# AdvancedPhotonSource/tike

Hardware: AMD Instinct MI355X
Metric: diffraction patterns/sec/GPU (256x256, 8-mode probe) (higher is better)
Workload: dtype c64; 1 GPU; c3; positions_per_gpu=10000, modes=8, detector=256, eigen_probes=1, solver=lstsq_grad, num_batch=10, chunk_positions=1000, position_correction=False, object_update=after every minibatch (batch_method wobbly_center), route=no_farplane

## Files before the change

include/tike_amd.h:

```cpp
#ifndef TIKE_AMD_H
#define TIKE_AMD_H

#ifdef __cplusplus
extern "C" {
#endif

#define TIKE_ERR_ARG 1000001
#define TIKE_ERR_UNSUPPORTED 1000002
#define TIKE_ERR_COMM 2000000
#define TIKE_COMM_ID_BYTES 128

#define TIKE_ABI_VERSION 14

const char* tike_build_id(void);

int tike_abi_version(void);

int tike_set_deterministic(int on, void* scratch, long bytes);

int tike_init(void);

int tike_patch_fwd(const void* images, void* patches, const float* positions, int nimage, int H,
                   int W, int nscan, int nrepeat, int patch_width, int padded_width,
                   void* stream);
int tike_patch_adj(void* images, const void* patches, const float* positions, int nimage, int H,
                   int W, int nscan, int nrepeat, int patch_width, int padded_width, int npatch,
                   void* stream);

int tike_conv_fwd(const void* psi, const float* scan, const void* probe, int probe_per_scan,
                  void* nearplane, int nscan, int S, int pw, int det, int H, int W, void* stream);
int tike_conv_adj(const void* nearplane, const float* scan, const void* probe,
                  int probe_per_scan, void* psi, int nscan, int S, int pw, int det, int H, int W,
                  void* stream);
int tike_conv_adj_probe(const void* nearplane, const float* scan, const void* psi,
                        void* probe_adj, int nscan, int S, int pw, int det, int H, int W,
                        void* stream);

int tike_fft2(const void* in, void* out, long ntile, int n, int inverse, float scale,
              void* stream);

int tike_fft2_supported(int n);

int tike_fft2_general(const void* in, void* out, long ntile, int n, int inverse, float scale,
                      int lines_per_group_rows, int lines_per_group_cols, void* stream);

int tike_ptycho_fwd(const void* psi, const float* scan, const void* probe, int probe_per_scan,
                    const void* eigen_probe, const float* eigen_weights, int num_eigen,
                    int eigen_modes, void* farplane, int nscan, int S, int pw, int det, int H,
                    int W, float scale, int sub_batch, void* stream);

int tike_ptycho_adj(const void* farplane, const void* probe, int probe_per_scan,
                    const float* scan, const void* psi, void* psi_adj, void* probe_adj,
                    void* objproj_work, float* acc_work, int nscan, int S, int pw, int det,
                    int H, int W, float scale, int sub_batch, void* stream);

int tike_ptycho_fwd_intensity(const void* psi, const float* scan, const void* probe,
                              int probe_per_scan, const void* unique_probe,
                              const float* eigen_weights, int num_eigen, int eigen_modes,
                              void* farplane, float* intensity, void* patches, int nscan, int S,
                              int pw, int det, int H, int W, float scale, void* stream);

int tike_ptycho_fwd_intensity_only(const void* psi, const float* scan, const void* probe,
                                   int probe_per_scan, const void* unique_probe,
                                   const float* eigen_weights, int num_eigen, int eigen_modes,
                                   void* scratch, float* intensity, int nscan, int S, int pw,
// ... 279 lines not shown
                                  const void* other, const float* scan, const void* data,
                                  int data_u16, void* far_a, int a_valid, void* far_b,
                                  float* costs_k, int nscan, int chunk, int S, int det, int H,
                                  int W, float fwd_scale, double count, double* state,
                                  int stage, double* sums, void* stream);

int tike_cgrad_line_search_linear_masked(int variable, const void* x, const void* d, void* xs,
                                         const void* other, const float* scan, const void* data,
                                         int data_u16, void* far_a, int a_valid, void* far_b,
                                         float* costs_k, int nscan, int chunk, int S, int det,
                                         int H, int W, float fwd_scale, double count,
                                         double* state, int stage, double* sums,
                                         const unsigned char* measured, int model,
                                         long num_measured, void* stream);

int tike_eigen_pixel_update1(const void* patches, const void* chi0, const void* mpu0,
                             const void* eigen0, const float* eigen_proj,
                             const float* weights_c, long weights_row, const float* norm,
                             void* update, int nscan, int pw, int chi_modes, const float* stats,
                             const float* costs, float eps, float* sums3, const void* psi,
                             const float* scan, int H, int W, void* stream);
int tike_lstsq_tail_mid(void* eigen0, const void* update, int npix, float* nacc,
                        float beta_eigen, const float* stats, int B, float eps,
                        const float* sums3, double count, int recover_psi, int recover_probe,
                        float* tail3, void* stream);
int tike_eigen_position_sums1(const void* patches, const void* chi0, const void* mpu0,
                              const void* eigen0, float* sums5, float* dsum, int nscan, int pw,
                              int chi_modes, const void* psi, const float* scan, int H, int W,
                              void* stream);
int tike_lstsq_tail_finish(const float* tail3, const float* sums3, double count, float* steps,
                           void* probe, void* combined, const void* mpu, float inv_num_batch,
                           long nprobe, float* weights, long weights_row, int S, int m,
                           const float* stats, const float* sums5, int B, int npix,
                           void* stream);

int tike_ifft2_pass2_gradients_eproj(const void* work, const void* patches, const void* probe,
                                     const void* eigen_probe, const float* eigen_weights,
                                     int num_eigen, int eigen_modes, void* objproj, void* chi0,
                                     void* m_probe_update, float mpu_scale, int nscan, int S,
                                     int det, float inv_scale, float* qtab, float* q,
                                     void* stream);
int tike_eigen_pixel_update1q(const void* patches, const void* chi0, const void* mpu0,
                              const void* eigen0, const float* q, const float* weights_c,
                              long weights_row, const float* norm, void* update, int nscan,
                              int pw, int chi_modes, const void* psi, const float* scan, int H,
                              int W, float* c0part, float* eproj_out, void* stream);
int tike_lstsq_step_stats_eigen1(const void* chi, const float* scan,
                                 const void* object_update_precond, const void* probe,
                                 const void* eigen_probe, const float* eigen_weights,
                                 int eigen_modes, const void* m_probe_update, const void* patches,
                                 const void* update, float* nacc, double count, float beta_eigen,
                                 float* stats, float* sums5, int nscan, int S, int chi_modes,
                                 int pw, int H, int W, void* stream);
int tike_lstsq_tail_solve1(void* eigen0, const void* update, int npix, const float* nacc,
                           float beta_eigen, const float* stats, const float* costs,
                           const float* sums5, int B, float eps, double count, int recover_psi,
                           int recover_probe, float* sums3, float* tail3, void* stream);

int tike_lstsq_chunk_gradients(const void* psi, const float* scan, const void* probe,
                               const void* eigen_probe, const float* eigen_weights,
                               int num_eigen, int eigen_modes, const void* data, int data_u16,
                               const unsigned char* measured, int model,
                               float unmeasured_scaling, long num_measured, void* scratch,
                               void* work, float* gscale, void* patches, float* costs,
                               void* objproj, void* chi0, void* m_probe_update,
                               float mpu_scale, float* object_acc, int nscan, int S, int det,
                               int H, int W, float fwd_scale, float inv_scale, void* stream);

int tike_comm_unique_id(void* id);
int tike_comm_create(const void* id, int nranks, int rank, void** comm);
int tike_comm_destroy(void* comm);
int tike_comm_allreduce_sum(void* comm, void* buf, long count, int f64, void* stream);
int tike_comm_broadcast(void* comm, void* buf, long nbytes, int root, void* stream);

int tike_cluster_farthest_fill(const float* points, long n, long* owner, int num_cluster,
                               long turns);
int tike_cluster_swap_sweep(const double* dist, long n, int k, long* label, const long* best,
                            const long* order, double* regret, int* moved);

#ifdef __cplusplus
}
#endif
#endif
```

tike_amd/_lib.py:

```python
import ctypes
import os
import re

import torch

_HERE = os.path.dirname(os.path.abspath(__file__))
LIB_PATH = os.environ.get("TIKE_AMD_LIB") or os.path.join(
    _HERE, "csrc", "libtike_amd.so")
HEADER_PATH = os.path.join(os.path.dirname(_HERE), "include", "tike_amd.h")

ABI_VERSION = 14
ERR_ARG = 1000001
ERR_UNSUPPORTED = 1000002
ERR_COMM = 2000000
COMM_ID_BYTES = 128

if not os.path.isfile(LIB_PATH):
    raise ImportError(
        f"{LIB_PATH} not found: build the HIP library first "
        "(`make -C tike_amd/csrc` or `python -c 'import __graft_entry__ as g; "
        "g.build()'`). tike_amd has no CPU fallback.")

lib = ctypes.CDLL(LIB_PATH)

_p = ctypes.c_void_p
_i = ctypes.c_int
_l = ctypes.c_long
_f = ctypes.c_float
_d = ctypes.c_double

_PROTOTYPES = {
    "tike_abi_version": [],
    "tike_init": [],
    "tike_set_deterministic": [_i, _p, _l],
    "tike_patch_fwd": [_p, _p, _p, _i, _i, _i, _i, _i, _i, _i, _p],
    "tike_patch_adj": [_p, _p, _p, _i, _i, _i, _i, _i, _i, _i, _i, _p],
    "tike_conv_fwd": [_p, _p, _p, _i, _p, _i, _i, _i, _i, _i, _i, _p],
    "tike_conv_adj": [_p, _p, _p, _i, _p, _i, _i, _i, _i, _i, _i, _p],
    "tike_conv_adj_probe": [_p, _p, _p, _p, _i, _i, _i, _i, _i, _i, _p],
    "tike_fft2": [_p, _p, _l, _i, _i, _f, _p],
    "tike_fft2_supported": [_i],
    "tike_fft2_general": [_p, _p, _l, _i, _i, _f, _i, _i, _p],
    "tike_pfa_supported": [_i, _i, _i],
    "tike_pfa_fwd_gather": [_p, _p, _p, _i, _p, _p, _p, _i, _i, _p, _p, _i, _i, _i,
                            _i, _i, _i, _p],
    "tike_pfa_fwd_subtiles_supported": [_i, _i, _i],
    "tike_pfa_fwd_subtiles": [_p, _p, _p, _p, _p, _i, _i, _p, _p, _p, _i, _i,
                              _i, _i, _i, _i, _p],
    "tike_pfa_fft2": [_p, _p, _l, _i, _i, _p],
    "tike_pfa_combine_gradient": [_p, _p, _p, _p, _i, _i, _i, _f, _i, _f, _l, _i,
                                  _p],
    "tike_pfa_inv_products": [_p, _p, _p, _i, _p, _p, _p, _i, _i, _p, _p, _p, _f,
                              _i, _i, _i, _i, _f, _p],
    "tike_gen_supported": [_i, _i, _i],
    "tike_gen_fwd_rows": [_p, _p, _p, _i, _p, _p, _p, _i, _i, _p, _p, _i, _i, _i,
                          _i, _i, _i, _p],
    "tike_gen_cols_gradient": [_p, _p, _p, _p, _p, _i, _i, _i, _i, _f, _i, _f,
                               _l, _p],
    "tike_gen_inv_rows_gradients": [_p, _p, _p, _i, _p, _p, _p, _i, _i, _p, _p,
                                    _p, _f, _i, _i, _i, _i, _f, _p],
    "tike_fresnel_spect_prop": [_p, _p, _p, _l, _i, _i, _f, _f, _p],
    "tike_fft2_pass1": [_p, _p, _l, _i, _i, _p],
    "tike_fft2_pass2_inplace": [_p, _l, _i, _i, _f, _p],
    "tike_slice_step": [_p, _p, _p, _p, _i, _i, _i, _i, _i, _f, _p],
# ... 39 lines not shown
    "tike_ifft2_pass2_gradients_modes": [_p, _p, _p, _p, _p, _i, _i, _p, _p,
                                         _p, _f, _i, _i, _i, _f, _i, _i, _i, _p],
    "tike_poisson_steps_grad_ifft2_pass1": [_p, _p, _i, _p, _p, _p, _p, _p, _i,
                                            _i, _i, _f, _f, _l, _f, _f, _p],
    "tike_object_update_precond": [_p, _p, _p, _f, _p, _p, _p, _l, _p],
    "tike_lstsq_step_sums": [_p, _p, _i, _f, _p, _p],
    "tike_lstsq_step_solve": [_p, _i, _f, _p, _d, _i, _i, _p, _p],
    "tike_probe_update": [_p, _p, _p, _p, _f, _l, _p],
    "tike_eigen_weights0": [_p, _p, _i, _i, _i, _i, _p, _p],
    "tike_eigen_proj_mean": [_p, _i, _p, _l, _p, _l, _i, _p, _p],
    "tike_eigen_normalise": [_p, _p, _d, _f, _i, _p, _p, _p],
    "tike_eigen_dsum": [_p, _i, _l, _p, _p],
    "tike_eigen_weights": [_p, _i, _l, _p, _d, _p, _l, _p, _i, _p, _p],
    "tike_grad_ifft2_crop": [_p, _p, _p, _p, _i, _p, _p, _l, _i, _i, _f, _f,
                             _p],
    "tike_position_sums": [_p, _p, _i, _p, _p, _p, _i, _i, _p, _i, _p, _p, _i,
                           _i, _i, _p],
    "tike_rpie_position_sums": [_p, _p, _p, _p, _i, _p, _p, _i, _i, _p, _i, _p,
                                _p, _p, _i, _i, _i, _i, _i, _p],
    "tike_farplane_gradient": [_p, _p, _p, _p, _p, _i, _i, _i, _i, _i, _f, _l,
                               _p],
    "tike_intensity": [_p, _p, _l, _i, _l, _p],
    "tike_cost_each_pattern": [_p, _p, _p, _l, _l, _i, _p],
    "tike_objective_grad": [_p, _p, _p, _p, _l, _i, _l, _i, _p],
    "tike_lstsq_gradients": [_p, _p, _p, _p, _p, _p, _i, _i, _p, _p, _p, _p, _i,
                             _i, _i, _i, _i, _p],
    "tike_varying_probe": [_p, _p, _p, _i, _i, _p, _i, _i, _i, _p],
    "tike_scatter_patches": [_p, _p, _p, _i, _i, _i, _i, _p],
    "tike_eigen_position_sums": [_p, _p, _p, _p, _p, _i, _i, _i, _p, _i, _i,
                                 _i, _p],
    "tike_eigen_pixel_update": [_p, _p, _p, _p, _p, _i, _i, _i, _p, _p, _i, _i,
                                _i, _p],
    "tike_probe_grad": [_p, _p, _p, _p, _p, _i, _i, _i, _i, _i, _p],
    "tike_probe_preconditioner": [_p, _p, _p, _i, _i, _i, _i, _p],
    "tike_psi_preconditioner": [_p, _p, _p, _i, _i, _i, _i, _p],
    "tike_scatter_amplitudes": [_p, _p, _p, _i, _i, _i, _i, _p],
    "tike_lstsq_step_stats": [_p, _p, _p, _p, _p, _p, _p, _i, _i, _p, _p, _p,
                              _p, _i, _i, _i, _i, _i, _i, _p, _p, _p],
    "tike_eigen_pixel_update1": [_p, _p, _p, _p, _p, _p, _l, _p, _p, _i, _i, _i,
                                 _p, _p, _f, _p, _p, _p, _i, _i, _p],
    "tike_lstsq_tail_mid": [_p, _p, _i, _p, _f, _p, _i, _f, _p, _d, _i, _i, _p,
                            _p],
    "tike_eigen_position_sums1": [_p, _p, _p, _p, _p, _p, _i, _i, _i, _p, _p,
                                  _i, _i, _p],
    "tike_lstsq_tail_finish": [_p, _p, _d, _p, _p, _p, _p, _f, _l, _p, _l, _i,
                               _i, _p, _p, _i, _i, _p],
    "tike_ifft2_pass2_gradients_eproj": [_p, _p, _p, _p, _p, _i, _i, _p, _p,
                                         _p, _f, _i, _i, _i, _f, _p, _p, _p],
    "tike_eigen_pixel_update1q": [_p, _p, _p, _p, _p, _p, _l, _p, _p, _i, _i,
                                  _i, _p, _p, _i, _i, _p, _p, _p],
    "tike_lstsq_step_stats_eigen1": [_p, _p, _p, _p, _p, _p, _i, _p, _p, _p,
                                     _p, _d, _f, _p, _p, _i, _i, _i, _i, _i,
                                     _i, _p],
    "tike_lstsq_tail_solve1": [_p, _p, _i, _p, _f, _p, _p, _p, _i, _f, _d, _i,
                               _i, _p, _p, _p],
    "tike_lstsq_chunk_gradients": [_p, _p, _p, _p, _p, _i, _i, _p, _i, _p, _i,
                                   _f, _l, _p, _p, _p, _p, _p, _p, _p, _p, _f,
                                   _p, _i, _i, _i, _i, _i, _f, _f, _p],
    "tike_cgrad_direction": [_p, _p, _p, _p, _l, _i, _p, _i, _d, _p, _p, _p],
    "tike_cgrad_line_search": [_i, _p, _p, _p, _p, _p, _p, _i, _p, _p, _i, _i,
                               _i, _i, _i, _i, _f, _d, _p, _p, _i, _p],
    "tike_cgrad_line_search_linear": [_i, _p, _p, _p, _p, _p, _p, _i, _p, _i, _p,
                                      _p, _i, _i, _i, _i, _i, _i, _f, _d, _p, _i,
                                      _p, _p],
    "tike_cgrad_line_search_masked": [_i, _p, _p, _p, _p, _p, _p, _i, _p, _p,
                                      _i, _i, _i, _i, _i, _i, _f, _d, _p, _p,
                                      _i, _p, _i, _l, _p],
    "tike_cgrad_line_search_linear_masked": [_i, _p, _p, _p, _p, _p, _p, _i, _p,
                                             _i, _p, _p, _i, _i, _i, _i, _i, _i,
                                             _f, _d, _p, _i, _p, _p, _i, _l, _p],
    "tike_comm_unique_id": [_p],
    "tike_comm_create": [_p, _i, _i, ctypes.POINTER(_p)],
    "tike_comm_destroy": [_p],
    "tike_comm_allreduce_sum": [_p, _p, _l, _i, _p],
    "tike_comm_broadcast": [_p, _p, _l, _i, _p],
    "tike_cluster_farthest_fill": [_p, _l, _p, _i, _l],
    "tike_cluster_swap_sweep": [_p, _l, _i, _p, _p, _p, _p, _p],
}


def build_id():
    try:
        fn = lib.tike_build_id
    except AttributeError:
        return ""
    fn.restype = ctypes.c_char_p
    fn.argtypes = []
    return fn().decode()


def declared_symbols():
    with open(HEADER_PATH) as f:
        text = f.read()
    return sorted(set(re.findall(r"^int\s+(tike_\w+)\s*\(", text, flags=re.M)))


for _name, _args in _PROTOTYPES.items():
    try:
        _fn = getattr(lib, _name)
    except AttributeError as e:
        raise ImportError(
            f"{LIB_PATH} does not export {_name}: it was built from another "
            "include/tike_amd.h; rebuild it (`make -C tike_amd/csrc`).") from e
    _fn.argtypes = _args
    _fn.restype = ctypes.c_int

# ... 48 lines not shown
```

tike_amd/csrc/lstsq.hip:

```cpp
#include "fft_engine2.h"
#include <type_traits>

#include "internal.h"
#include "tike_amd.h"

#ifndef TK_STATS_PAIRS
#define TK_STATS_PAIRS 1
#endif
static const bool g_stats_pairs = TK_STATS_PAIRS != 0;

constexpr int TK_STRIP = 32;
#define TK_ATOMIC_ADD(p, v) unsafeAtomicAdd(p, v)

template <bool REAL_ONLY, class ValueFn, class Sink>
__device__ __forceinline__ void scatter_footprint_rows(ValueFn&& value, float fx, float fy,
                                                       int pw, int r0, int r1, Sink&& sink) {
  for (int x0 = 0; x0 < pw; x0 += blockDim.x) {
    const int xp = x0 + threadIdx.x;
    const bool active = xp < pw;
    cf uprev = mk(0.f, 0.f), uprev_last = mk(0.f, 0.f);
    constexpr int RG = 4;
    cf vv[RG], ll[RG], nv[RG], nl[RG];
    auto load_group = [&](int yb, cf (&a)[RG], cf (&b)[RG]) {
      const int xpc = active ? xp : pw - 1;
// ... 1812 lines not shown
  auto taps16 = [&](const unsigned off) {
    tk_v4f t;
    __builtin_memcpy(&t, reinterpret_cast<const char*>(psi) + off, sizeof(t));
    return t;
  };
  auto tap = [](const tk_v4f u, const tk_v4f l, const TkCorner& c) {
    cf o = mk(u.x * c.w00, u.y * c.w00);
    o.x += u.z * c.w01;
    o.y += u.w * c.w01;
    o.x += l.x * c.w10;
    o.y += l.y * c.w10;
    o.x += l.z * c.w11;
    o.y += l.w * c.w11;
    return o;
  };
  for (int pair = blockIdx.x; pair < npair; pair += gridDim.x) {
    const int n0 = 2 * pair;
    const bool two = n0 + 1 < nscan;
    const TkCorner c0 = tk_corner(scan, n0);
    const TkCorner c1 = tk_corner(scan, two ? n0 + 1 : n0);
    const bool in0 = tk_interior(c0, pw, H, W), in1 = tk_interior(c1, pw, H, W);
    if (!(two && in0 && in1)) {
      one(n0, c0, in0);
      if (two) one(n0 + 1, c1, in1);
      continue;
    }
    float a[5] = {0.f, 0.f, 0.f, 0.f, 0.f}, b[5] = {0.f, 0.f, 0.f, 0.f, 0.f};
    const unsigned base0 = (unsigned)(c0.sy * W + c0.sx), base1 = (unsigned)(c1.sy * W + c1.sx);
    const cf* __restrict__ chi_a = R.chi0 + (long)n0 * R.XS;
    const cf* __restrict__ chi_b = chi_a + R.XS;
    const int ybeg = ((int)threadIdx.x / cols) * rows;
    for (int x = (int)threadIdx.x % cols; x < pw; x += 256) {
      unsigned rel = (unsigned)(ybeg * W + x);
      tk_v4f u0 = taps16((base0 + rel) * 8u), u1 = taps16((base1 + rel) * 8u);
      int p = ybeg * pw + x;
#pragma unroll 2
      for (int y = 0; y < rows; ++y) {
        rel += (unsigned)W;
        const tk_v4f l0 = taps16((base0 + rel) * 8u), l1 = taps16((base1 + rel) * 8u);
        const cf e = E[p], m0 = R.mpu0[p];
        const cf xa = chi_a[p], xb = chi_b[p];
        add(a, tap(u0, l0, c0), xa, e, m0);
        add(b, tap(u1, l1, c1), xb, e, m0);
        u0 = l0;
        u1 = l1;
        p += pw;
      }
    }
    finish(a, n0);
    finish(b, n0 + 1);
  }
}

__global__ __launch_bounds__(256) __attribute__((amdgpu_waves_per_eu(4)))
void step_stats_eigen_pair_kernel(
    const cf* __restrict__ chi, const float* __restrict__ scan, const cf* __restrict__ gobj,
    const TkProbe probe, const cf* __restrict__ mpu, const cf* __restrict__ patches,
    const cf* __restrict__ update, const float* __restrict__ nacc, float inv_count, float beta,
    float* __restrict__ stats, float* __restrict__ sums5, int nscan, int chi_modes, int pw,
    int H, int W, int nsplit) {
  __shared__ float red[4];
  typedef float tk_v4f __attribute__((ext_vector_type(4)));
  const long P = (long)pw * pw;
  const int plen = (int)(P / nsplit);
  const int npair = (nscan + 1) / 2;
  const float uu = nacc[0], ee = nacc[1], eu = nacc[2];
  const float mu = sqrtf(uu * inv_count * inv_count / (float)P);
  const float kk = beta / mu * inv_count;
  const float inv = 1.0f / sqrtf((ee + 2.0f * kk * eu + kk * kk * uu) / (float)P);
  auto enew = [&](const cf e, const long p) { return (e + update[p] * kk) * inv; };
  auto esum = [](float* a, const cf o, const cf x, const cf e, const cf m0) {
    const cf r = conjf(o) * x - m0;
    const cf phi = o * e;
    a[0] += r.x * e.x + r.y * e.y;
    a[1] += x.x * phi.x + x.y * phi.y;
    a[2] += norm2(phi);
    a[3] += r.y * e.x - r.x * e.y;
  };
  auto put = [&](float* dst, const float v) {
    if (nsplit > 1)
      unsafeAtomicAdd(dst, v);
    else
      *dst = v;
  };
  auto finish5 = [&](const float* a, const int n) {
    float t[4];
#pragma unroll
    for (int k = 0; k < 4; ++k) t[k] = tk_block_sum256(a[k], red);
    if (threadIdx.x == 0) {
      float* o = sums5 + (long)n * 5;
      put(o, t[0]);
      put(o + 1, t[1]);
      put(o + 2, t[2]);
      put(o + 3, t[0]);
      put(o + 4, t[3]);
    }
  };
  for (int v = blockIdx.x; v < npair * nsplit; v += gridDim.x) {
    const int n0 = 2 * (v / nsplit), part = v % nsplit;
    const TkCorner c0 = tk_corner(scan, n0);
    const bool two = n0 + 1 < nscan;
    const TkCorner c1 = tk_corner(scan, two ? n0 + 1 : n0);
    const bool in0 = c0.sy >= 0 && c0.sx >= 0 && c0.sy + pw < H && c0.sx + pw < W;
    const bool in1 = c1.sy >= 0 && c1.sx >= 0 && c1.sy + pw < H && c1.sx + pw < W;
    const int pbeg = part * plen + (int)threadIdx.x;
    const int pend = part + 1 == nsplit ? (int)P : (part + 1) * plen;
    if (!(two && in0 && in1)) {
      for (int i = 0; i < (two ? 2 : 1); ++i) {
        const int n = n0 + i;
        step_stats_item<true, true>(chi, scan, nullptr, gobj, probe, mpu, patches, stats,
                                    chi_modes, pw, H, W, nullptr, nullptr, nsplit, n, part, red);
        float a[4] = {0.f, 0.f, 0.f, 0.f};
        for (int p = pbeg; p < pend; p += blockDim.x)
          esum(a, patches[(long)n * P + p], chi[(long)n * chi_modes * P + p],
               enew(probe.eigen[p], p), mpu[p]);
        finish5(a, n);
      }
      continue;
    }
    float s0 = 1.0f, s1 = 1.0f, t0 = 0.f, t1 = 0.f;
    if (probe.weights != nullptr) {
      const float* w = probe.weights + n0 * (long)(probe.C + 1) * probe.S;
      s0 = w[0];
      s1 = w[(long)(probe.C + 1) * probe.S];
      t0 = w[probe.S];
      t1 = w[(long)(probe.C + 1) * probe.S + probe.S];
    }
    float a[8] = {0.f, 0.f, 0.f, 0.f, 0.f, 0.f, 0.f, 0.f};
    float b[8] = {0.f, 0.f, 0.f, 0.f, 0.f, 0.f, 0.f, 0.f};
    float ea[4] = {0.f, 0.f, 0.f, 0.f}, eb[4] = {0.f, 0.f, 0.f, 0.f};
    const unsigned base0 = (unsigned)(c0.sy * W + c0.sx), base1 = (unsigned)(c1.sy * W + c1.sx);
    const cf* __restrict__ chi_a = chi + ((long)n0 * chi_modes) * P;
    const cf* __restrict__ chi_b = chi + ((long)(n0 + 1) * chi_modes) * P;
    const cf* __restrict__ pat_a = patches + (long)n0 * P;
    const cf* __restrict__ pat_b = pat_a + P;
    auto tap = [](const tk_v4f u, const tk_v4f l, const TkCorner& c) {
      cf g = mk(u.x * c.w00, u.y * c.w00);
      g.x += u.z * c.w01;
      g.y += u.w * c.w01;
      g.x += l.x * c.w10;
      g.y += l.y * c.w10;
      g.x += l.z * c.w11;
      g.y += l.w * c.w11;
      return g;
    };
    auto sums = [](float* acc, const cf g, const cf o, const cf x0, const cf p0, const cf pn,
                   const cf m0) {
      const cf dOP = g * pn;
      const cf dPO = m0 * o;
      const cf OP = o * p0;
      acc[0] += norm2(dOP);
      acc[1] += norm2(dPO);
      const cf a2 = dOP * conjf(dPO);
      acc[2] += a2.x;
      acc[3] += a2.y;
      acc[4] += dOP.x * x0.x + dOP.y * x0.y;
      acc[5] += dPO.x * x0.x + dPO.y * x0.y;
      acc[6] += OP.x * x0.x + OP.y * x0.y;
      acc[7] += norm2(OP);
    };
    auto pixel = [&](const int p, const tk_v4f u0, const tk_v4f l0, const tk_v4f u1,
                     const tk_v4f l1) {
      const cf oa = pat_a[p], ob = pat_b[p];
      const cf xa = chi_a[p], xb = chi_b[p];
      const cf p0 = probe.probe[p];
      const cf m0 = mpu[p];
      const cf e1 = probe.eigen[p];
      const cf en = enew(e1, p);
      cf pa = p0 * s0, pb = p0 * s1;
      pa.x += t0 * e1.x;
      pa.y += t0 * e1.y;
      pb.x += t1 * e1.x;
      pb.y += t1 * e1.y;
      sums(a, tap(u0, l0, c0), oa, xa, p0, pa, m0);
      sums(b, tap(u1, l1, c1), ob, xb, p0, pb, m0);
      esum(ea, oa, xa, en, m0);
      esum(eb, ob, xb, en, m0);
    };
    auto taps16 = [&](const unsigned off) {
      tk_v4f t;
      __builtin_memcpy(&t, reinterpret_cast<const char*>(gobj) + off, sizeof(t));
      return t;
    };
    const int cols = pw < 256 ? pw : 256, groups = 256 / cols;
    const int rows = pw / (nsplit * groups);
    const int ybeg = (part * groups + (int)threadIdx.x / cols) * rows;
    for (int x = (int)threadIdx.x % cols; x < pw; x += 256) {
      unsigned rel = (unsigned)(ybeg * W + x);
      tk_v4f u0 = taps16((base0 + rel) * 8u), u1 = taps16((base1 + rel) * 8u);
      int p = ybeg * pw + x;
#pragma unroll 2
      for (int y = 0; y < rows; ++y) {
        rel += (unsigned)W;
        const tk_v4f l0 = taps16((base0 + rel) * 8u), l1 = taps16((base1 + rel) * 8u);
        pixel(p, u0, l0, u1, l1);
        u0 = l0;
        u1 = l1;
        p += pw;
      }
    }
#pragma unroll
    for (int k = 0; k < 8; ++k) {
      const float ta = tk_block_sum256(a[k], red);
      const float tb = tk_block_sum256(b[k], red);
      if (threadIdx.x == 0) {
        put(&stats[(long)n0 * 8 + k], ta);
        put(&stats[(long)n0 * 8 + 8 + k], tb);
      }
    }
    finish5(ea, n0);
    finish5(eb, n0 + 1);
  }
}

__global__ __launch_bounds__(256) void eigen_norm_sums1_kernel(const cf* __restrict__ E,
                                                               const cf* __restrict__ update,
                                                               int npix, float* __restrict__ nacc,
                                                               float* __restrict__ part) {
  __shared__ float red[4];
  float uu = 0.f, ee = 0.f, eu = 0.f;
  for (int i = blockIdx.x * 256 + threadIdx.x; i < npix; i += gridDim.x * 256) {
    const cf e = E[i], u = update[i];
    uu += norm2(u);
    ee += norm2(e);
    eu += e.x * u.x + e.y * u.y;
  }
  uu = tk_block_sum256(uu, red);
  ee = tk_block_sum256(ee, red);
  eu = tk_block_sum256(eu, red);
  if (threadIdx.x == 0) {
    if (part != nullptr) {
      part[3 * blockIdx.x] = uu;
      part[3 * blockIdx.x + 1] = ee;
      part[3 * blockIdx.x + 2] = eu;
    } else {
      unsafeAtomicAdd(&nacc[0], uu);
      unsafeAtomicAdd(&nacc[1], ee);
      unsafeAtomicAdd(&nacc[2], eu);
    }
  }
}

extern "C" int tike_lstsq_step_stats_eigen1(const void* chi, const float* scan,
                                            const void* object_update_precond, const void* probe,
                                            const void* eigen_probe, const float* eigen_weights,
                                            int eigen_modes, const void* m_probe_update,
                                            const void* patches, const void* update, float* nacc,
                                            double count, float beta_eigen, float* stats,
                                            float* sums5, int nscan, int S, int chi_modes,
                                            int pw, int H, int W, void* stream) {
  TK_ENTER();
  TK_CHECK_ARG(nscan >= 0 && S >= 1 && chi_modes >= 1 && pw >= 1 && H >= 1 && W >= 1 &&
               eigen_modes >= 1 && count > 0);
  TK_CHECK_ARG(probe && eigen_probe && eigen_weights && m_probe_update && update && nacc);
  const long P = (long)pw * pw;
  const long nitem = (nscan + 1) / 2;
  int nsplit = 1;
  while (nsplit < 16 && nitem * nsplit * 2 <= 8192 && P % (2048L * nsplit) == 0) nsplit *= 2;
  if (tk_deterministic()) nsplit = 1;
  const int groups = 256 / (pw < 256 ? pw : 256);
  if (!((pw % 256 == 0 || 256 % pw == 0) && pw % (nsplit * groups) == 0 &&
        (long)H * W < (1L << 28)))
    return TK_ERR_UNSUPPORTED;
  int grid = P >= 256 * 64 ? 64 : (int)((P + 255) / 256);
  float* part = nullptr;
  if (tk_deterministic()) {
    part = tk_det_scratch(sizeof(float) * 3 * (size_t)grid);
    if (part == nullptr) grid = 1;
  }
  hipLaunchKernelGGL(eigen_norm_sums1_kernel, dim3(grid), dim3(256), 0, (hipStream_t)stream,
                     (const cf*)eigen_probe, (const cf*)update, (int)P, nacc, part);
  TK_LAUNCH_CHECK();
  if (part != nullptr) {
    int rc = tk_ordered_sum(nacc, part, 3, grid, true, (hipStream_t)stream);
    if (rc) return rc;
  }
  if (nscan == 0) return TK_OK;
  TK_CHECK_ARG(chi && scan && object_update_precond && patches && stats && sums5);
  const TkProbe pr = tk_make_probe(probe, 0, eigen_probe, eigen_weights, 1, eigen_modes, S, pw,
                                   nullptr);
  if (nsplit > 1) {
    hipError_t e = hipMemsetAsync(stats, 0, sizeof(float) * 8 * (size_t)nscan, (hipStream_t)stream);
    if (e == hipSuccess)
      e = hipMemsetAsync(sums5, 0, sizeof(float) * 5 * (size_t)nscan, (hipStream_t)stream);
    if (e != hipSuccess) return (int)e;
  }
  hipLaunchKernelGGL(step_stats_eigen_pair_kernel, dim3(tk_grid(nitem * nsplit, 16)), dim3(256),
                     0, (hipStream_t)stream, (const cf*)chi, scan,
                     (const cf*)object_update_precond, pr, (const cf*)m_probe_update,
                     (const cf*)patches, (const cf*)update, (const float*)nacc,
                     (float)(1.0 / count), beta_eigen, stats, sums5, nscan, chi_modes, pw, H, W,
                     nsplit);
  TK_LAUNCH_CHECK();
  return TK_OK;
}

static TkResidual make_residual(const void* patches, const void* chi0, const void* mpu0,
                                const void* eigen, const void* coefs, int C, int Sm, int c,
                                int pw, int chi_modes) {
  TkResidual R;
  R.patches = (const cf*)patches;
  R.chi0 = (const cf*)chi0;
  R.mpu0 = (const cf*)mpu0;
  R.eigen = (const cf*)eigen;
  R.coefs = (const cf*)coefs;
  R.C = C;
  R.Sm = Sm;
  R.c = c;
  R.P = (long)pw * pw;
  R.XS = R.P * chi_modes;
  return R;
}

extern "C" int tike_eigen_position_sums(const void* patches, const void* chi0, const void* mpu0,
                                        const void* eigen_probe, const void* coefs,
                                        int num_eigen, int eigen_modes, int c, float* sums,
                                        int nscan, int pw, int chi_modes, void* stream) {
  TK_ENTER();
  TK_CHECK_ARG(nscan >= 0 && pw >= 1 && num_eigen >= 1 && c >= 0 && c < num_eigen &&
               chi_modes >= 1);
  if (nscan == 0) return TK_OK;
  TK_CHECK_ARG(patches && chi0 && mpu0 && eigen_probe && sums && (c == 0 || coefs));
  const TkResidual R = make_residual(patches, chi0, mpu0, eigen_probe, coefs, num_eigen,
                                     eigen_modes, c, pw, chi_modes);
  if (c == 0)
    hipLaunchKernelGGL(eigen_position_sums_kernel<true>, dim3(tk_grid(nscan, 16)), dim3(256), 0,
                       (hipStream_t)stream, R, sums, nscan);
  else
    hipLaunchKernelGGL(eigen_position_sums_kernel<false>, dim3(tk_grid(nscan, 16)), dim3(256),
                       0, (hipStream_t)stream, R, sums, nscan);
  TK_LAUNCH_CHECK();
  return TK_OK;
}

extern "C" int tike_eigen_pixel_update(const void* patches, const void* chi0, const void* mpu0,
                                       const void* eigen_probe, const void* coefs,
                                       int num_eigen, int eigen_modes, int c, const float* pm,
                                       void* update, int nscan, int pw, int chi_modes,
                                       void* stream) {
  TK_ENTER();
  TK_CHECK_ARG(nscan >= 0 && pw >= 1 && num_eigen >= 1 && c >= 0 && c < num_eigen &&
               chi_modes >= 1);
  if (nscan == 0) return TK_OK;
  TK_CHECK_ARG(patches && chi0 && mpu0 && eigen_probe && pm && update && (c == 0 || coefs));
  const long P = (long)pw * pw;
  float* part = nullptr;
  const int chunk = probe_chunk(nscan, 2 * P, &part);
// ... 606 lines not shown
```

tike_amd/ptycho/solvers/lstsq.py:

```python
import logging
from types import SimpleNamespace

import numpy as np
import torch

from ... import _arrays as A
from ... import _tuning
from ... import linalg
from ... import opt
from ... import random as trandom
from ..._lib import check, lib
from ...operators.propagation import fft_scales
from ..position import gaussian_derivative_taps
from ._plan import GradientPlan

logger = logging.getLogger(__name__)

_MODELS = {"gaussian": 0, "poisson": 1}


class _Workspace:

    def __init__(self):
        self.buffers = {}
# ... 645 lines not shown
            lib.tike_eigen_position_sums1(
                A.ptr(g["patches"]), A.ptr(g["chi0"]), A.ptr(mpu[0, 0, 0]),
                A.ptr(E), A.ptr(sums5), tail3[2:].data_ptr(), B, pw,
                g["chi_modes"], gpsi if EIGEN_SUMS_RECOMPUTE else None,
                A.ptr(scan[lo:hi]), psi.shape[-2], psi.shape[-1], st),
            "eigen position sums")
    if comm.collective:
        comm.Allreduce(tail3)
    check(
        lib.tike_lstsq_tail_finish(
            A.ptr(tail3), A.ptr(sums3), count, A.ptr(steps_row),
            A.ptr(probe) if recover_probe else None,
            A.ptr(probe_combined_update) if recover_probe else None,
            A.ptr(mpu), 1.0 / num_batch, probe.numel(),
            None if w_rows is None else w_rows.data_ptr(), row, S, 0,
            A.ptr(stats), A.ptr(sums5), B, P, st), "minibatch tail")
    return (steps_row[2] if recover_psi else None,
            steps_row[3] if recover_probe else None)


def _fused_tail(g, psi, scan, probe, eigen_probe, eigen_weights,
                object_update_precond, lo, hi, *, op, num_batch, recover_psi,
                recover_probe, norm, steps_row, probe_combined_update, sums3,
                update, nacc, tail3):
    B = hi - lo
    dev = psi.device
    st = A.stream_ptr()
    S, pw = probe.shape[-3], probe.shape[-1]
    P = pw * pw
    H, W = psi.shape[-2:]
    count = float(g["count"])
    ws = _workspace(op)
    mpu = g["m_probe_update"]
    Sm = eigen_probe.shape[-3]
    w_rows = eigen_weights[lo:hi]
    row = w_rows.shape[-2] * w_rows.shape[-1]
    E = eigen_probe[0, 0, 0]
    eps_total = float(np.float32(np.float32(1e-9) / P) * P)
    stats = ws.get("stats", (max(B, 1), 8), torch.float32, dev)
    sums5 = ws.get("eigen_sums5", (max(B, 1), 5), torch.float32, dev)
    eproj = ws.get("eigen_proj", (max(B, 1),), torch.float32, dev)
    c0part = ws.get("eigen_c0part", (64,), torch.float32, dev)
    g["eigen_proj"] = eproj[:B]
    gpsi = A.ptr(psi[0]) if EIGEN_PATCH_RECOMPUTE else None
    scan_b = A.ptr(scan[lo:hi])
    check(
        lib.tike_eigen_pixel_update1q(
            A.ptr(g["patches"]), A.ptr(g["chi0"]), A.ptr(mpu[0, 0, 0]),
            A.ptr(E), A.ptr(g["q"]), w_rows[:, 1, 0].data_ptr(), row,
            A.ptr(norm), A.ptr(update), B, pw, g["chi_modes"], gpsi, scan_b,
            H, W, A.ptr(c0part), A.ptr(eproj), st),
        "eigen pixel update")
    beta_eigen = min(0.1, 1.0 / num_batch)
    check(
        lib.tike_lstsq_step_stats_eigen1(
            A.ptr(g["chi0"]), scan_b, A.ptr(object_update_precond),
            A.ptr(probe), A.ptr(eigen_probe), A.ptr(g["w_old"]), Sm,
            A.ptr(mpu), A.ptr(g["patches"]), A.ptr(update), A.ptr(nacc), count,
            beta_eigen, A.ptr(stats), A.ptr(sums5), B, S, g["chi_modes"], pw,
            H, W, st),
        "step-size statistics + eigen position sums")
    check(
        lib.tike_lstsq_tail_solve1(
            A.ptr(E), A.ptr(update), P, A.ptr(nacc), beta_eigen, A.ptr(stats),
            A.ptr(g["costs"]), A.ptr(sums5), B, eps_total, count,
            int(recover_psi), int(recover_probe), A.ptr(sums3), A.ptr(tail3),
            st), "eigen probe + step solve")
    check(
        lib.tike_lstsq_tail_finish(
            A.ptr(tail3), A.ptr(sums3), count, A.ptr(steps_row),
            A.ptr(probe) if recover_probe else None,
            A.ptr(probe_combined_update) if recover_probe else None,
            A.ptr(mpu), 1.0 / num_batch, probe.numel(), w_rows.data_ptr(), row,
            S, 0, A.ptr(stats), A.ptr(sums5), B, P, st), "minibatch tail")
    g["stats"] = stats[:B]
    g["sums5"] = sums5[:B]
    return (steps_row[2] if recover_psi else None,
            steps_row[3] if recover_probe else None)


def _solve_steps(stats, costs, count, comm, *, pw, recover_psi, recover_probe,
                 out=None):
    dev = stats.device
    B = stats.shape[0]
    st = A.stream_ptr()
    eps_total = float(np.float32(np.float32(1e-9) / (pw * pw)) * (pw * pw))
    if out is None:
        out = torch.zeros(5, dtype=torch.float32, device=dev)
    sums = torch.empty(3, dtype=torch.float32, device=dev)
    check(
        lib.tike_lstsq_step_sums(A.ptr(stats), A.ptr(costs), B, eps_total,
                                 A.ptr(sums), st), "step-size sums")
    if comm.collective:
        comm.Allreduce(sums)
    check(
        lib.tike_lstsq_step_solve(A.ptr(stats), B, eps_total, A.ptr(sums),
                                  float(count), int(recover_psi),
                                  int(recover_probe), A.ptr(out), st),
        "step-size solve")
    if comm.collective:
        comm.Allreduce(out[:2])
        out[2:4] = out[:2] / count
    return (out[2] if recover_psi else None,
            out[3] if recover_probe else None, out[4])


def _update_nearplane(g, stats, probe, eigen_probe, eigen_weights, lo, hi,
                      comm, *, num_batch):
    m = 0
    dev = probe.device
    count = float(g["count"])
    B = hi - lo
    st = A.stream_ptr()
# ... 119 lines not shown
```

Measured before the change: 217,400 patterns/s.

## Split step-stats eigen kernel into strip-parallel pass with DPP reduction and finish kernel

Adds a strip kernel in which each block owns a horizontal strip of the probe and loops over a chunk of scan positions. Per-pixel step statistics and eigen sums are kept in registers and reduced across the wave with DPP and shuffles. Each wave writes 16 partial slots per position to a workspace table, and a second finish kernel sums those partials into stats and sums5. Positions that fall out of bounds go through the old per-item path. This trades the pair kernel's full-patch-per-block scheme and its atomics or memset for better parallelism and reuse of probe registers, at the cost of an extra launch and a workspace buffer.

```diff
diff --git a/include/tike_amd.h b/include/tike_amd.h
--- a/include/tike_amd.h
+++ b/include/tike_amd.h
@@ -10,7 +10,7 @@
 #define TIKE_ERR_COMM 2000000
 #define TIKE_COMM_ID_BYTES 128
 
-#define TIKE_ABI_VERSION 14
+#define TIKE_ABI_VERSION 15
 
 const char* tike_build_id(void);
 
@@ -396,6 +396,15 @@
                                  const void* update, float* nacc, double count, float beta_eigen,
                                  float* stats, float* sums5, int nscan, int S, int chi_modes,
                                  int pw, int H, int W, void* stream);
+int tike_lstsq_step_stats_eigen1w(const void* chi, const float* scan,
+                                  const void* object_update_precond, const void* probe,
+                                  const void* eigen_probe, const float* eigen_weights,
+                                  int eigen_modes, const void* m_probe_update,
+                                  const void* patches, const void* update, float* nacc,
+                                  double count, float beta_eigen, float* stats, float* sums5,
+                                  int nscan, int S, int chi_modes, int pw, int H, int W,
+                                  float* work, long work_floats, void* stream);
+int tike_lstsq_step_stats_strips_work(int nscan, int pw);
 int tike_lstsq_tail_solve1(void* eigen0, const void* update, int npix, const float* nacc,
                            float beta_eigen, const float* stats, const float* costs,
                            const float* sums5, int B, float eps, double count, int recover_psi,
diff --git a/tike_amd/_lib.py b/tike_amd/_lib.py
--- a/tike_amd/_lib.py
+++ b/tike_amd/_lib.py
@@ -9,7 +9,7 @@
     _HERE, "csrc", "libtike_amd.so")
 HEADER_PATH = os.path.join(os.path.dirname(_HERE), "include", "tike_amd.h")
 
-ABI_VERSION = 14
+ABI_VERSION = 15
 ERR_ARG = 1000001
 ERR_UNSUPPORTED = 1000002
 ERR_COMM = 2000000
@@ -155,6 +155,10 @@
     "tike_lstsq_step_stats_eigen1": [_p, _p, _p, _p, _p, _p, _i, _p, _p, _p,
                                      _p, _d, _f, _p, _p, _i, _i, _i, _i, _i,
                                      _i, _p],
+    "tike_lstsq_step_stats_eigen1w": [_p, _p, _p, _p, _p, _p, _i, _p, _p, _p,
+                                      _p, _d, _f, _p, _p, _i, _i, _i, _i, _i,
+                                      _i, _p, _l, _p],
+    "tike_lstsq_step_stats_strips_work": [_i, _i],
     "tike_lstsq_tail_solve1": [_p, _p, _i, _p, _f, _p, _p, _p, _i, _f, _d, _i,
                                _i, _p, _p, _p],
     "tike_lstsq_chunk_gradients": [_p, _p, _p, _p, _p, _i, _i, _p, _i, _p, _i,
diff --git a/tike_amd/csrc/lstsq.hip b/tike_amd/csrc/lstsq.hip
--- a/tike_amd/csrc/lstsq.hip
+++ b/tike_amd/csrc/lstsq.hip
@@ -1888,6 +1888,54 @@
   }
 }
 
+typedef float tk_v4f __attribute__((ext_vector_type(4)));
+struct TkEigenScale {
+  float kk, inv;
+};
+__device__ __forceinline__ TkEigenScale tk_eigen_scale(const float* __restrict__ nacc,
+                                                       float inv_count, float beta, long P) {
+  const float uu = nacc[0], ee = nacc[1], eu = nacc[2];
+  const float mu = sqrtf(uu * inv_count * inv_count / (float)P);
+  TkEigenScale s;
+  s.kk = beta / mu * inv_count;
+  s.inv = 1.0f / sqrtf((ee + 2.0f * s.kk * eu + s.kk * s.kk * uu) / (float)P);
+  return s;
+}
+__device__ __forceinline__ cf tk_tap16(const tk_v4f u, const tk_v4f l, const TkCorner& c) {
+  cf g = mk(u.x * c.w00, u.y * c.w00);
+  g.x += u.z * c.w01;
+  g.y += u.w * c.w01;
+  g.x += l.x * c.w10;
+  g.y += l.y * c.w10;
+  g.x += l.z * c.w11;
+  g.y += l.w * c.w11;
+  return g;
+}
+__device__ __forceinline__ void tk_stats_pixel(float* acc, const cf g, const cf o, const cf x0,
+                                               const cf p0, const cf pn, const cf m0) {
+  const cf dOP = g * pn;
+  const cf dPO = m0 * o;
+  const cf OP = o * p0;
+  acc[0] += norm2(dOP);
+  acc[1] += norm2(dPO);
+  const cf a2 = dOP * conjf(dPO);
+  acc[2] += a2.x;
+  acc[3] += a2.y;
+  acc[4] += dOP.x * x0.x + dOP.y * x0.y;
+  acc[5] += dPO.x * x0.x + dPO.y * x0.y;
+  acc[6] += OP.x * x0.x + OP.y * x0.y;
+  acc[7] += norm2(OP);
+}
+__device__ __forceinline__ void tk_esum_pixel(float* a, const cf o, const cf x, const cf e,
+                                              const cf m0) {
+  const cf r = conjf(o) * x - m0;
+  const cf phi = o * e;
+  a[0] += r.x * e.x + r.y * e.y;
+  a[1] += x.x * phi.x + x.y * phi.y;
+  a[2] += norm2(phi);
+  a[3] += r.y * e.x - r.x * e.y;
+}
+
 __global__ __launch_bounds__(256) __attribute__((amdgpu_waves_per_eu(4)))
 void step_stats_eigen_pair_kernel(
     const cf* __restrict__ chi, const float* __restrict__ scan, const cf* __restrict__ gobj,
@@ -1896,22 +1944,14 @@
     float* __restrict__ stats, float* __restrict__ sums5, int nscan, int chi_modes, int pw,
     int H, int W, int nsplit) {
   __shared__ float red[4];
-  typedef float tk_v4f __attribute__((ext_vector_type(4)));
   const long P = (long)pw * pw;
   const int plen = (int)(P / nsplit);
   const int npair = (nscan + 1) / 2;
-  const float uu = nacc[0], ee = nacc[1], eu = nacc[2];
-  const float mu = sqrtf(uu * inv_count * inv_count / (float)P);
-  const float kk = beta / mu * inv_count;
-  const float inv = 1.0f / sqrtf((ee + 2.0f * kk * eu + kk * kk * uu) / (float)P);
+  const TkEigenScale es = tk_eigen_scale(nacc, inv_count, beta, P);
+  const float kk = es.kk, inv = es.inv;
   auto enew = [&](const cf e, const long p) { return (e + update[p] * kk) * inv; };
   auto esum = [](float* a, const cf o, const cf x, const cf e, const cf m0) {
-    const cf r = conjf(o) * x - m0;
-    const cf phi = o * e;
-    a[0] += r.x * e.x + r.y * e.y;
-    a[1] += x.x * phi.x + x.y * phi.y;
-    a[2] += norm2(phi);
-    a[3] += r.y * e.x - r.x * e.y;
+    tk_esum_pixel(a, o, x, e, m0);
   };
   auto put = [&](float* dst, const float v) {
     if (nsplit > 1)
@@ -1970,31 +2010,6 @@
     const cf* __restrict__ chi_b = chi + ((long)(n0 + 1) * chi_modes) * P;
     const cf* __restrict__ pat_a = patches + (long)n0 * P;
     const cf* __restrict__ pat_b = pat_a + P;
-    auto tap = [](const tk_v4f u, const tk_v4f l, const TkCorner& c) {
-      cf g = mk(u.x * c.w00, u.y * c.w00);
-      g.x += u.z * c.w01;
-      g.y += u.w * c.w01;
-      g.x += l.x * c.w10;
-      g.y += l.y * c.w10;
-      g.x += l.z * c.w11;
-      g.y += l.w * c.w11;
-      return g;
-    };
-    auto sums = [](float* acc, const cf g, const cf o, const cf x0, const cf p0, const cf pn,
-                   const cf m0) {
-      const cf dOP = g * pn;
-      const cf dPO = m0 * o;
-      const cf OP = o * p0;
-      acc[0] += norm2(dOP);
-      acc[1] += norm2(dPO);
-      const cf a2 = dOP * conjf(dPO);
-      acc[2] += a2.x;
-      acc[3] += a2.y;
-      acc[4] += dOP.x * x0.x + dOP.y * x0.y;
-      acc[5] += dPO.x * x0.x + dPO.y * x0.y;
-      acc[6] += OP.x * x0.x + OP.y * x0.y;
-      acc[7] += norm2(OP);
-    };
     auto pixel = [&](const int p, const tk_v4f u0, const tk_v4f l0, const tk_v4f u1,
                      const tk_v4f l1) {
       const cf oa = pat_a[p], ob = pat_b[p];
@@ -2008,8 +2023,8 @@
       pa.y += t0 * e1.y;
       pb.x += t1 * e1.x;
       pb.y += t1 * e1.y;
-      sums(a, tap(u0, l0, c0), oa, xa, p0, pa, m0);
-      sums(b, tap(u1, l1, c1), ob, xb, p0, pb, m0);
+      tk_stats_pixel(a, tk_tap16(u0, l0, c0), oa, xa, p0, pa, m0);
+      tk_stats_pixel(b, tk_tap16(u1, l1, c1), ob, xb, p0, pb, m0);
       esum(ea, oa, xa, en, m0);
       esum(eb, ob, xb, en, m0);
     };
@@ -2049,6 +2064,169 @@
   }
 }
 
+constexpr int TK_STAT_SLOTS = 16;
+
+template <int CTL>
+__device__ __forceinline__ float tk_dpp(float x) {
+  return __int_as_float(__builtin_amdgcn_update_dpp(0, __float_as_int(x), CTL, 0xf, 0xf, false));
+}
+
+__device__ __forceinline__ float tk_strip_reduce(const float* v, int lane) {
+  const bool b3 = lane & 8, b2 = lane & 4, b1 = lane & 2, b0 = lane & 1;
+  float w[8];
+#pragma unroll
+  for (int i = 0; i < 8; ++i) {
+    const float hi = i < 4 ? v[8 + i] : 0.f;
+    const float keep = b3 ? hi : v[i], send = b3 ? v[i] : hi;
+    w[i] = keep + tk_dpp<0x140>(send);
+  }
+#pragma unroll
+  for (int i = 0; i < 4; ++i) {
+    const float keep = b2 ? w[4 + i] : w[i], send = b2 ? w[i] : w[4 + i];
+    w[i] = keep + tk_dpp<0x141>(send);
+  }
+#pragma unroll
+  for (int i = 0; i < 2; ++i) {
+    const float keep = b1 ? w[2 + i] : w[i], send = b1 ? w[i] : w[2 + i];
+    w[i] = keep + tk_dpp<0x4e>(send);
+  }
+  const float keep = b0 ? w[1] : w[0], send = b0 ? w[0] : w[1];
+  float r = keep + tk_dpp<0xb1>(send);
+  r += __shfl_xor(r, 16, 64);
+  r += __shfl_xor(r, 32, 64);
+  return r;
+}
+
+template <int R>
+__global__ __launch_bounds__(256) __attribute__((amdgpu_waves_per_eu(4)))
+void step_stats_eigen_strip_kernel(
+    const cf* __restrict__ chi, const float* __restrict__ scan, const cf* __restrict__ gobj,
+    const TkProbe probe, const cf* __restrict__ mpu, const cf* __restrict__ patches,
+    const cf* __restrict__ update, const float* __restrict__ nacc, float inv_count, float beta,
+    float* __restrict__ tab, int nscan, int chi_modes, int pw, int H, int W, int chunk) {
+  const long P = (long)pw * pw;
+  const int cols = pw, groups = 256 / cols;
+  const int nstrip = pw / (groups * R);
+  const int strip = (int)blockIdx.x % nstrip, ch = (int)blockIdx.x / nstrip;
+  const int x = (int)threadIdx.x % cols;
+  const int ybeg = (strip * groups + (int)threadIdx.x / cols) * R;
+  const int lane = (int)threadIdx.x & 63, wave = (int)threadIdx.x >> 6;
+  const TkEigenScale es = tk_eigen_scale(nacc, inv_count, beta, P);
+  cf p0[R], m0[R], e1[R], en[R];
+#pragma unroll
+  for (int y = 0; y < R; ++y) {
+    const int p = (ybeg + y) * pw + x;
+    p0[y] = probe.probe[p];
+    m0[y] = mpu[p];
+    e1[y] = probe.eigen[p];
+    en[y] = (e1[y] + update[p] * es.kk) * es.inv;
+  }
+  auto taps16 = [&](const unsigned off) {
+    tk_v4f t;
+    __builtin_memcpy(&t, reinterpret_cast<const char*>(gobj) + off, sizeof(t));
+    return t;
+  };
+  auto opaque = [&]() {
+#pragma unroll
+    for (int y = 0; y < R; ++y)
+      asm volatile("" : "+v"(p0[y].x), "+v"(p0[y].y), "+v"(m0[y].x), "+v"(m0[y].y),
+                        "+v"(e1[y].x), "+v"(e1[y].y), "+v"(en[y].x), "+v"(en[y].y));
+  };
+  opaque();
+  const int nend = (ch + 1) * chunk < nscan ? (ch + 1) * chunk : nscan;
+  const long wstride = (long)(probe.C + 1) * probe.S;
+  const unsigned rel0 = (unsigned)(ybeg * W + x);
+  const unsigned pix0 = (unsigned)(ybeg * pw + x);
+  for (int n = ch * chunk; n < nend; ++n) {
+    const TkCorner c = tk_corner(scan, n);
+    if (!(c.sy >= 0 && c.sx >= 0 && c.sy + pw < H && c.sx + pw < W)) continue;
+    const float* __restrict__ w = probe.weights + n * wstride;
+    const float s0 = w[0], t0 = w[probe.S];
+    const unsigned base = (unsigned)(c.sy * W + c.sx);
+    const cf* __restrict__ chi_n = chi + ((long)n * chi_modes) * P;
+    const cf* __restrict__ pat_n = patches + (long)n * P;
+    opaque();
+    unsigned poff = pix0 * 8u;
+    asm volatile("" : "+v"(poff));
+    tk_v4f t[R + 1];
+    cf o[R], x0[R];
+#pragma unroll
+    for (int y = 0; y <= R; ++y) t[y] = taps16((base + rel0 + (unsigned)(y * W)) * 8u);
+#pragma unroll
+    for (int y = 0; y < R; ++y) {
+      o[y] = *tk_at(pat_n, poff + (unsigned)(y * pw) * 8u);
+      x0[y] = *tk_at(chi_n, poff + (unsigned)(y * pw) * 8u);
+    }
+    float v[12];
+#pragma unroll
+    for (int k = 0; k < 12; ++k) v[k] = 0.f;
+#pragma unroll
+    for (int y = 0; y < R; ++y) {
+      cf pn = p0[y] * s0;
+      pn.x += t0 * e1[y].x;
+      pn.y += t0 * e1[y].y;
+      tk_stats_pixel(v, tk_tap16(t[y], t[y + 1], c), o[y], x0[y], p0[y], pn, m0[y]);
+      tk_esum_pixel(v + 8, o[y], x0[y], en[y], m0[y]);
+    }
+    const float r = tk_strip_reduce(v, lane);
+    if (lane < TK_STAT_SLOTS)
+      tab[(((long)n * nstrip + strip) * 4 + wave) * TK_STAT_SLOTS + lane] = r;
+  }
+}
+
+__global__ __launch_bounds__(256) void step_stats_strip_finish_kernel(
+    const float* __restrict__ tab, int nslab, const cf* __restrict__ chi,
+    const float* __restrict__ scan, const cf* __restrict__ gobj, const TkProbe probe,
+    const cf* __restrict__ mpu, const cf* __restrict__ patches, const cf* __restrict__ update,
+    const float* __restrict__ nacc, float inv_count, float beta, float* __restrict__ stats,
+    float* __restrict__ sums5, int nscan, int chi_modes, int pw, int H, int W) {
+  __shared__ float red[4];
+  __shared__ float part[16][TK_STAT_SLOTS];
+  const long P = (long)pw * pw;
+  for (int n = blockIdx.x; n < nscan; n += gridDim.x) {
+    const TkCorner c = tk_corner(scan, n);
+    if (!(c.sy >= 0 && c.sx >= 0 && c.sy + pw < H && c.sx + pw < W)) {
+      const TkEigenScale es = tk_eigen_scale(nacc, inv_count, beta, P);
+      step_stats_item<true, true>(chi, scan, nullptr, gobj, probe, mpu, patches, stats,
+                                  chi_modes, pw, H, W, nullptr, nullptr, 1, n, 0, red);
+      float a[4] = {0.f, 0.f, 0.f, 0.f};
+      for (int p = threadIdx.x; p < (int)P; p += 256)
+        tk_esum_pixel(a, patches[(long)n * P + p], chi[(long)n * chi_modes * P + p],
+                      (probe.eigen[p] + update[p] * es.kk) * es.inv, mpu[p]);
+      float t[4];
+#pragma unroll
+      for (int k = 0; k < 4; ++k) t[k] = tk_block_sum256(a[k], red);
+      if (threadIdx.x == 0) {
+        float* o = sums5 + (long)n * 5;
+        o[0] = t[0];
+        o[1] = t[1];
+        o[2] = t[2];
+        o[3] = t[0];
+        o[4] = t[3];
+      }
+      continue;
+    }
+    const int slot = (int)threadIdx.x & 15, g = (int)threadIdx.x >> 4;
+    float s = 0.f;
+    for (int k = g; k < nslab; k += 16) s += tab[((long)n * nslab + k) * TK_STAT_SLOTS + slot];
+    __syncthreads();
+    part[g][slot] = s;
+    __syncthreads();
+    if (threadIdx.x < 12) {
+      float t = 0.f;
+#pragma unroll
+      for (int k = 0; k < 16; ++k) t += part[k][slot];
+      if (slot < 8) {
+        stats[(long)n * 8 + slot] = t;
+      } else {
+        float* o = sums5 + (long)n * 5;
+        o[slot < 11 ? slot - 8 : 4] = t;
+        if (slot == 8) o[3] = t;
+      }
+    }
+  }
+}
+
 __global__ __launch_bounds__(256) void eigen_norm_sums1_kernel(const cf* __restrict__ E,
                                                                const cf* __restrict__ update,
                                                                int npix, float* __restrict__ nacc,
@@ -2077,14 +2255,29 @@
   }
 }
 
-extern "C" int tike_lstsq_step_stats_eigen1(const void* chi, const float* scan,
-                                            const void* object_update_precond, const void* probe,
-                                            const void* eigen_probe, const float* eigen_weights,
-                                            int eigen_modes, const void* m_probe_update,
-                                            const void* patches, const void* update, float* nacc,
-                                            double count, float beta_eigen, float* stats,
-                                            float* sums5, int nscan, int S, int chi_modes,
-                                            int pw, int H, int W, void* stream) {
+#ifndef TK_STAT_STRIP_ROWS
+#define TK_STAT_STRIP_ROWS 4
+#endif
+static inline int tk_stat_strips(int pw) {
+  if (pw < 1 || pw > 256 || 256 % pw != 0) return 0;
+  const int rows = (256 / pw) * TK_STAT_STRIP_ROWS;
+  return pw % rows == 0 ? pw / rows : 0;
+}
+
+extern "C" int tike_lstsq_step_stats_strips_work(int nscan, int pw) {
+  const long n = (long)nscan * tk_stat_strips(pw) * 4 * TK_STAT_SLOTS;
+  return nscan < 1 || n > 0x7fffffffL ? 0 : (int)n;
+}
+
+extern "C" int tike_lstsq_step_stats_eigen1w(const void* chi, const float* scan,
+                                             const void* object_update_precond, const void* probe,
+                                             const void* eigen_probe, const float* eigen_weights,
+                                             int eigen_modes, const void* m_probe_update,
+                                             const void* patches, const void* update, float* nacc,
+                                             double count, float beta_eigen, float* stats,
+                                             float* sums5, int nscan, int S, int chi_modes,
+                                             int pw, int H, int W, float* work, long work_floats,
+                                             void* stream) {
   TK_ENTER();
   TK_CHECK_ARG(nscan >= 0 && S >= 1 && chi_modes >= 1 && pw >= 1 && H >= 1 && W >= 1 &&
                eigen_modes >= 1 && count > 0);
@@ -2115,6 +2308,27 @@
   TK_CHECK_ARG(chi && scan && object_update_precond && patches && stats && sums5);
   const TkProbe pr = tk_make_probe(probe, 0, eigen_probe, eigen_weights, 1, eigen_modes, S, pw,
                                    nullptr);
+  const int need = tike_lstsq_step_stats_strips_work(nscan, pw);
+  if (work != nullptr && need > 0 && work_floats >= need) {
+    const int nstrip = tk_stat_strips(pw);
+    int chunk = (int)(((long)nscan * nstrip + 2047) / 2048);
+    chunk = chunk < 1 ? 1 : (chunk > 128 ? 128 : chunk);
+    const int nchunk = (nscan + chunk - 1) / chunk;
+    hipLaunchKernelGGL(step_stats_eigen_strip_kernel<TK_STAT_STRIP_ROWS>, dim3(nchunk * nstrip),
+                       dim3(256), 0, (hipStream_t)stream, (const cf*)chi, scan,
+                       (const cf*)object_update_precond, pr, (const cf*)m_probe_update,
+                       (const cf*)patches, (const cf*)update, (const float*)nacc,
+                       (float)(1.0 / count), beta_eigen, work, nscan, chi_modes, pw, H, W, chunk);
+    TK_LAUNCH_CHECK();
+    hipLaunchKernelGGL(step_stats_strip_finish_kernel, dim3(tk_grid(nscan, 8)), dim3(256), 0,
+                       (hipStream_t)stream, (const float*)work, nstrip * 4, (const cf*)chi, scan,
+                       (const cf*)object_update_precond, pr, (const cf*)m_probe_update,
+                       (const cf*)patches, (const cf*)update, (const float*)nacc,
+                       (float)(1.0 / count), beta_eigen, stats, sums5, nscan, chi_modes, pw, H,
+                       W);
+    TK_LAUNCH_CHECK();
+    return TK_OK;
+  }
   if (nsplit > 1) {
     hipError_t e = hipMemsetAsync(stats, 0, sizeof(float) * 8 * (size_t)nscan, (hipStream_t)stream);
     if (e == hipSuccess)
@@ -2129,6 +2343,20 @@
                      nsplit);
   TK_LAUNCH_CHECK();
   return TK_OK;
+}
+
+extern "C" int tike_lstsq_step_stats_eigen1(const void* chi, const float* scan,
+                                            const void* object_update_precond, const void* probe,
+                                            const void* eigen_probe, const float* eigen_weights,
+                                            int eigen_modes, const void* m_probe_update,
+                                            const void* patches, const void* update, float* nacc,
+                                            double count, float beta_eigen, float* stats,
+                                            float* sums5, int nscan, int S, int chi_modes,
+                                            int pw, int H, int W, void* stream) {
+  return tike_lstsq_step_stats_eigen1w(chi, scan, object_update_precond, probe, eigen_probe,
+                                       eigen_weights, eigen_modes, m_probe_update, patches,
+                                       update, nacc, count, beta_eigen, stats, sums5, nscan, S,
+                                       chi_modes, pw, H, W, nullptr, 0, stream);
 }
 
 static TkResidual make_residual(const void* patches, const void* chi0, const void* mpu0,
diff --git a/tike_amd/ptycho/solvers/lstsq.py b/tike_amd/ptycho/solvers/lstsq.py
--- a/tike_amd/ptycho/solvers/lstsq.py
+++ b/tike_amd/ptycho/solvers/lstsq.py
@@ -721,13 +721,15 @@
             H, W, A.ptr(c0part), A.ptr(eproj), st),
         "eigen pixel update")
     beta_eigen = min(0.1, 1.0 / num_batch)
-    check(
-        lib.tike_lstsq_step_stats_eigen1(
+    nwork = lib.tike_lstsq_step_stats_strips_work(B, pw)
+    work = ws.get("stats_strips", (max(nwork, 1),), torch.float32, dev)
+    check(
+        lib.tike_lstsq_step_stats_eigen1w(
             A.ptr(g["chi0"]), scan_b, A.ptr(object_update_precond),
             A.ptr(probe), A.ptr(eigen_probe), A.ptr(g["w_old"]), Sm,
             A.ptr(mpu), A.ptr(g["patches"]), A.ptr(update), A.ptr(nacc), count,
             beta_eigen, A.ptr(stats), A.ptr(sums5), B, S, g["chi_modes"], pw,
-            H, W, st),
+            H, W, A.ptr(work), nwork, st),
         "step-size statistics + eigen position sums")
     check(
         lib.tike_lstsq_tail_solve1(
```

After: 219,100 patterns/s (median of 4 runs). No clear change (+0.8%).
